# ivanalberico/End-To-End-Self-Supervised-SLAM

Hardware: AMD Instinct MI355X
Metric: online refinement steps/sec @640x480, seq_len=60 (higher is better)
Workload: dtype f32

## Files before the change

end-to-end-self-supervised-slam_amd/csrc/conv.hip:

```cpp
#include <cassert>
#include <type_traits>

#include "e2e_common.h"

typedef float f4v __attribute__((ext_vector_type(4)));
typedef float f16v __attribute__((ext_vector_type(16)));

#define CBK 16

enum { ACT_NONE = 0, ACT_RELU = 1, ACT_ELU = 2, ACT_DISP = 3 };

struct ConvArgs {
    const float* src0;
    const float* src1;
    const float* w;
    const float* scale;
    const float* shift;
    const float* res;
    float* out;
    int B, Hs, Ws;
    int Cin, C1, up;
    int Hd, Wd;
    int Ncols, ldw;
    int KH, KW, stride, pad, pad_mode;
    int off;
    int act;
    float in_sub, in_mul;
    int ksplit, cps;
    float* slab;
    int cls;
    const float* xin;
    int dact;
    const float* pre;
    int64_t cls_rows;
    int64_t bytes0, bytes1, bytesw;
};

__device__ __forceinline__ float apply_act(float v, int act) {
    if (act == ACT_RELU) return fmaxf(v, 0.f);
    if (act == ACT_ELU) return v > 0.f ? v : expm1f(v);
    if (act == ACT_DISP) return 10.f / (1.f + expf(-v)) + 0.01f;
    return v;
}

__device__ __forceinline__ float act_deriv(float y, int act) {
    if (act == ACT_RELU) return y > 0.f ? 1.f : 0.f;
    if (act == ACT_ELU) return y > 0.f ? 1.f : y + 1.f;
    return 1.f;
}

template <bool TRANSPOSED>
__device__ __forceinline__ bool tap_coord(const ConvArgs& a, int yd, int xd, int kh, int kw, int& ys, int& xs) {
    if (!TRANSPOSED) {
        ys = yd * a.stride + kh - a.pad;
        xs = xd * a.stride + kw - a.pad;
        if (a.pad_mode == 1) {
            ys = reflect1(ys, a.Hs);
            xs = reflect1(xs, a.Ws);
// ... 821 lines not shown
    float wreg[9][KQ];
#pragma unroll
    for (int t = 0; t < 9; ++t)
#pragma unroll
        for (int j = 0; j < KQ; ++j) wreg[t][j] = a.w[(int64_t)((a.flip ? 8 - t : t) * CIN + 4 * j + kq) * a.ldw + l16];
    const float* sb = a.src + (int64_t)b * a.Hsrc * a.Wsrc * CIN;
    for (int idx = tid; idx < PH * PW * KQ; idx += 256) {
        const int q = (UP == 2) ? idx / (PH * PW) : idx % KQ, pix = (UP == 2) ? idx % (PH * PW) : idx / KQ;
        const int py = pix / PW, px = pix - py * PW;
        int Y = y0 - a.org + py, X = x0 - a.org + px;
        bool ok = true;
        if (REFLECT) {
            Y = min(max(reflect1(Y, HD), 0), HD - 1);
            X = min(max(reflect1(X, WD), 0), WD - 1);
        } else {
            ok = Y >= 0 && Y < HD && X >= 0 && X < WD;
        }
        f4v v = {0.f, 0.f, 0.f, 0.f};
        if (ok) v = *(const f4v*)(sb + ((int64_t)(Y / UP) * a.Wsrc + (X / UP)) * CIN + q * 4);
#pragma unroll
        for (int e = 0; e < 4; ++e) patch[(q * 4 + e) * PLANE + py * PWS + px] = v[e];
    }
    __syncthreads();
    const float bv = a.bias ? a.bias[l16] : 0.f;
    float* ob = a.out + (int64_t)b * a.Hd * a.Wd * 16;
#pragma unroll 1
    for (int g2 = 0; g2 < TH; g2 += 2) {
        const int g0 = wave * TH + g2, g1 = g0 + 1;
        const int r0 = g0 >> 2, c0 = (g0 & 3) * 16, r1 = g1 >> 2, c1 = (g1 & 3) * 16;
        f4v acc0 = {0.f, 0.f, 0.f, 0.f}, acc1 = {0.f, 0.f, 0.f, 0.f};
        const float* p0 = patch + kq * PLANE + r0 * PWS + c0 + l16;
        const float* p1 = patch + kq * PLANE + r1 * PWS + c1 + l16;
#pragma unroll
        for (int t = 0; t < 9; ++t) {
            const int off = (t / 3) * PWS + (t % 3);
#pragma unroll
            for (int j = 0; j < KQ; ++j) {
                acc0 = __builtin_amdgcn_mfma_f32_16x16x4f32(p0[4 * j * PLANE + off], wreg[t][j], acc0, 0, 0, 0);
                acc1 = __builtin_amdgcn_mfma_f32_16x16x4f32(p1[4 * j * PLANE + off], wreg[t][j], acc1, 0, 0, 0);
            }
        }
#pragma unroll
        for (int h = 0; h < 2; ++h) {
            const f4v acc = h ? acc1 : acc0;
            const int y = y0 + (h ? r1 : r0), xb = x0 + (h ? c1 : c0) + 4 * kq;
            if (y >= a.Hd) continue;
#pragma unroll
            for (int i = 0; i < 4; ++i)
                if (xb + i < a.Wd) ob[((int64_t)y * a.Wd + xb + i) * 16 + l16] = apply_act(acc[i] + bv, a.act);
        }
    }
}

struct StemArgs {
    const float* src;
    const float* w;
    const float* scale;
    const float* shift;
    float* out;
    int B, Hs, Ws, Hd, Wd, ldw, act;
    float in_sub, in_mul;
};

__global__ __launch_bounds__(256) void k_conv7x7_stem(StemArgs a) {
    constexpr int TH = 4, TW = 32, PH = 2 * TH + 6, PW = 2 * TW + 5, ROW = 208, NJ = 37;
    __shared__ float patch[PH * ROW];
    const int tid = threadIdx.x, lane = tid & 63, wave = tid >> 6, l16 = lane & 15, kq = lane >> 4;
    const int x0 = blockIdx.x * TW, y0 = blockIdx.y * TH, b = blockIdx.z;
    const int co = 16 * wave + l16;
    float wreg[NJ];
    int offk[NJ];
#pragma unroll
    for (int j = 0; j < NJ; ++j) {
        const int k = 4 * j + kq;
        wreg[j] = k < 147 ? a.w[(int64_t)k * a.ldw + co] : 0.f;
        offk[j] = k + (k / 21) * (ROW - 21);
    }
    const float* sb = a.src + (int64_t)b * a.Hs * a.Ws * 3;
    for (int idx = tid; idx < PH * ROW; idx += 256) {
        const int py = idx / ROW, e = idx - py * ROW;
        const int Y = 2 * y0 - 3 + py, X = 2 * x0 - 3 + e / 3;
        const bool ok = e < 3 * PW && Y >= 0 && Y < a.Hs && X >= 0 && X < a.Ws;
        patch[idx] = ok ? (sb[((int64_t)Y * a.Ws + X) * 3 + (e - (e / 3) * 3)] - a.in_sub) * a.in_mul : 0.f;
    }
    __syncthreads();
    const float sc = a.scale ? a.scale[co] : 1.f, sh = a.shift ? a.shift[co] : 0.f;
    float* ob = a.out + (int64_t)b * a.Hd * a.Wd * 64;
#pragma unroll 1
    for (int g = 0; g < 2 * TH; g += 2) {
        const int r = g >> 1;
        const float* p0 = patch + 2 * r * ROW + 6 * l16;
        const float* p1 = p0 + 6 * 16;
        f4v acc0 = {0.f, 0.f, 0.f, 0.f}, acc1 = {0.f, 0.f, 0.f, 0.f};
#pragma unroll
        for (int j = 0; j < NJ; ++j) {
            acc0 = __builtin_amdgcn_mfma_f32_16x16x4f32(p0[offk[j]], wreg[j], acc0, 0, 0, 0);
            acc1 = __builtin_amdgcn_mfma_f32_16x16x4f32(p1[offk[j]], wreg[j], acc1, 0, 0, 0);
        }
        const int y = y0 + r;
        if (y >= a.Hd) continue;
#pragma unroll
        for (int h = 0; h < 2; ++h) {
            const f4v acc = h ? acc1 : acc0;
            const int xb = x0 + 16 * h + 4 * kq;
#pragma unroll
            for (int i = 0; i < 4; ++i)
// ... 1850 lines not shown
}

int64_t e2e_conv_tuned_workspace_floats(int64_t rows, int cols) {
    int64_t n = (int64_t)16 * rows * cols;
    if (n < (int64_t)SK_MAX_G * 64 * 64) n = (int64_t)SK_MAX_G * 64 * 64;
    return n + SK_FLAG_FLOATS;
}
int e2e_conv_workspace_flag_floats(void) { return SK_FLAG_FLOATS; }
int e2e_conv_streamk_error_index(void) { return SK_ERR_INDEX; }

int e2e_conv_gemm_choice(int64_t rows, int cols, int K, int chunk_depth, int allow_split, int* out3) {
    E2E_REQUIRE(out3 && rows > 0 && cols > 0 && K > 0 && (chunk_depth == 16 || chunk_depth == 32), E2E_ERR_ARG, "e2e_conv_gemm_choice: bad argument");
    const GemmCfg c = choose_cfg(rows, cols, K, chunk_depth, allow_split != 0);
    out3[0] = c.bm; out3[1] = c.bn; out3[2] = c.S;
    return E2E_OK;
}

struct ConvGeom { int B, Hs, Ws, Cin, Cout, Ho, Wo, KH, KW, stride, pad, pad_mode, C1, up; float in_sub, in_mul; };
#define GEOM_LAYER(g) ConvGeom g{}; g.B = B; g.Hs = Hs; g.Ws = Ws; g.Cin = Cin; g.Cout = Cout; g.KH = KH; g.KW = KW; g.stride = stride; g.pad = pad; g.pad_mode = pad_mode
#define GEOM_SOURCES(g) g.C1 = C1; g.up = up; g.in_sub = in_sub; g.in_mul = in_mul
#define GEOM_OUTPUT(g) g.Ho = Ho; g.Wo = Wo
#define GEOM_BWD_DATA(g) GEOM_LAYER(g); GEOM_OUTPUT(g)
#define GEOM_BWD_WEIGHT(g) GEOM_LAYER(g); GEOM_OUTPUT(g); GEOM_SOURCES(g)
#define GEOM_WGRAD_QUERY(g) ConvGeom g{}; g.B = B; g.Ho = Ho; g.Wo = Wo; g.Cin = Cin; g.Cout = Cout; g.KH = KH; g.KW = KW
struct FwdOps { const float *src0, *src1, *w_fwd; int ld_fwd; const float *scale, *shift, *residual; float* out; int act; };
struct BwdDataOps { const float* dz; const float* w_bwd; int ld_bwd; float* dxp; int accumulate; const float* x_in; int in_act; const float* pre_add; };
struct WgradIn { const float *dz, *src0, *src1; float* workspace; };

static int fwd_setup(const FwdOps& f, const ConvGeom& g, ConvArgs& a_out, int& vec_out, const char* who) {
    const int B = g.B, Hs = g.Hs, Ws = g.Ws, Cin = g.Cin, Cout = g.Cout, KH = g.KH, KW = g.KW, stride = g.stride, pad = g.pad, pad_mode = g.pad_mode;
    const int C1 = g.C1, up = g.up, ld_fwd = f.ld_fwd;
    E2E_REQUIRE(f.src0 && f.w_fwd && f.out && B > 0 && Hs > 0 && Ws > 0 && Cin > 0 && Cout > 0 && KH > 0 && KW > 0, E2E_ERR_ARG, "%s: bad argument", who);
    E2E_REQUIRE(up == 1 || up == 2, E2E_ERR_ARG, "%s: upsample factor must be 1 or 2", who);
    E2E_REQUIRE(C1 > 0 && C1 <= Cin && (C1 == Cin || f.src1), E2E_ERR_ARG, "%s: bad channel split", who);
    E2E_REQUIRE(pad_mode == 0 || (pad_mode == 1 && pad == 1 && Hs >= 2 && Ws >= 2), E2E_ERR_ARG, "%s: reflection padding needs pad == 1", who);
    E2E_REQUIRE(stride == 1 || stride == 2, E2E_ERR_ARG, "%s: stride must be 1 or 2", who);
    E2E_REQUIRE(Hs % up == 0 && Ws % up == 0 && ld_fwd % 4 == 0 && ld_fwd >= Cout, E2E_ERR_ARG, "%s: bad sizes", who);
    E2E_REQUIRE(pad >= 0 && Hs + 2 * pad >= KH && Ws + 2 * pad >= KW, E2E_ERR_ARG, "%s: the kernel must fit the padded input (pad >= 0)", who);
    const int vec = (Cin % 16 == 0 && (C1 == Cin || C1 % 16 == 0)) ? 4 : 1;
    E2E_REQUIRE(vec == 4 || (C1 == Cin && up == 1), E2E_ERR_ARG, "%s: the scalar path (Cin %% 16 != 0) takes a single full-resolution source", who);
    E2E_REQUIRE((int64_t)B * Hs * Ws * Cin * 4 < (1ll << 30) && (int64_t)KH * KW * Cin * ld_fwd * 4 < (1ll << 31), E2E_ERR_ARG,
                "%s: activations must stay below 1 GB, weights below 2 GB (32-bit buffer offsets with out-of-range markers)", who);
    E2E_REQUIRE(vec != 4 || (KH <= 3 && KW <= 3), E2E_ERR_ARG, "%s: the channel-quad loader takes kernels up to 3 x 3", who);
    ConvArgs a{};
    a.src0 = f.src0; a.src1 = f.src1; a.w = f.w_fwd; a.scale = f.scale; a.shift = f.shift; a.res = f.residual; a.out = f.out;
    a.B = B; a.Hs = Hs; a.Ws = Ws; a.Cin = Cin; a.C1 = C1; a.up = up;
    a.Hd = (Hs + 2 * pad - KH) / stride + 1; a.Wd = (Ws + 2 * pad - KW) / stride + 1;
    a.Ncols = Cout; a.ldw = ld_fwd; a.KH = KH; a.KW = KW; a.stride = stride; a.pad = pad; a.pad_mode = pad_mode; a.off = 0; a.act = f.act;
    a.in_sub = g.in_sub; a.in_mul = g.in_mul;
    a_out = a; vec_out = vec;
    return E2E_OK;
}

static int conv_fwd_impl(const FwdOps& f, const ConvGeom& g, float* workspace, GemmCfg force, void* stream) {
    const int B = g.B, Hs = g.Hs, Ws = g.Ws, Cin = g.Cin, Cout = g.Cout, KH = g.KH, KW = g.KW, stride = g.stride, pad = g.pad, pad_mode = g.pad_mode;
    const int C1 = g.C1, up = g.up, ld_fwd = f.ld_fwd;
    ConvArgs a;
    int vec;
    const int rc = fwd_setup(f, g, a, vec, "e2e_conv2d_fwd");
    if (rc != E2E_OK) return rc;
    if (!force.bm && KH == 7 && KW == 7 && stride == 2 && pad == 3 && pad_mode == 0 && Cin == 3 && Cout == 64 && C1 == Cin && up == 1 && !f.residual && ld_fwd >= 64) {
        StemArgs t{f.src0, f.w_fwd, f.scale, f.shift, f.out, B, Hs, Ws, a.Hd, a.Wd, ld_fwd, f.act, g.in_sub, g.in_mul};
        hipLaunchKernelGGL(k_conv7x7_stem, dim3((a.Wd + 31) / 32, (a.Hd + 3) / 4, B), dim3(256), 0, (hipStream_t)stream, t);
    }
    else if (!force.bm && KH == 3 && KW == 3 && stride == 1 && pad == 1 && pad_mode == 1 && Cout == 16 && C1 == Cin && !f.scale && !f.residual && ld_fwd >= 16 &&
        ((Cin == 16 && up == 2) || (Cin == 32 && up == 1))) {
        ThinArgs t{f.src0, f.w_fwd, f.shift, f.out, B, Hs / up, Ws / up, Hs, Ws, ld_fwd, f.act, 1, 0};
        if (Cin == 16) hipLaunchKernelGGL((k_conv3x3_thin<16, 2, true, 8>), dim3((Ws + 63) / 64, (Hs + 7) / 8, B), dim3(256), 0, (hipStream_t)stream, t);
        else hipLaunchKernelGGL((k_conv3x3_thin<32, 1, true, 4>), dim3((Ws + 63) / 64, (Hs + 3) / 4, B), dim3(256), 0, (hipStream_t)stream, t);
    } else
        launch_gemm<false>(a, vec, workspace, force, (hipStream_t)stream);
    E2E_LAUNCH_CHECK("e2e_conv2d_fwd");
    return E2E_OK;
}

int e2e_conv2d_fwd(const float* src0, const float* src1, int C1, int up, const float* w_fwd, int ld_fwd, const float* scale,
                   const float* shift, const float* residual, float* out, int B, int Hs, int Ws, int Cin, int Cout, int KH,
                   int KW, int stride, int pad, int pad_mode, int act, float in_sub, float in_mul, float* workspace, void* stream) {
    GEOM_LAYER(g); GEOM_SOURCES(g);
    return conv_fwd_impl(FwdOps{src0, src1, w_fwd, ld_fwd, scale, shift, residual, out, act}, g, workspace, GemmCfg{0, 0, 0}, stream);
}

static bool tuning_ok(int tile_m, int tile_n, int ksplit) {
    if (tile_m == 0) return true;
    if (ksplit < 0) return tile_m == 64 && tile_n == 64 && -ksplit <= SK_MAX_G;
    return tile_max_cb(tile_m, tile_n) != 0 && ksplit >= 1 && ksplit <= 16;
}

int e2e_conv2d_fwd_tuned(const float* src0, const float* src1, int C1, int up, const float* w_fwd, int ld_fwd, const float* scale,
                         const float* shift, const float* residual, float* out, int B, int Hs, int Ws, int Cin, int Cout, int KH,
                         int KW, int stride, int pad, int pad_mode, int act, float in_sub, float in_mul, float* workspace, int tile_m, int tile_n,
                         int ksplit, void* stream) {
    E2E_REQUIRE(tuning_ok(tile_m, tile_n, ksplit), E2E_ERR_ARG, "e2e_conv2d_fwd_tuned: unsupported decomposition %d x %d / %d", tile_m, tile_n, ksplit);
    GEOM_LAYER(g); GEOM_SOURCES(g);
    return conv_fwd_impl(FwdOps{src0, src1, w_fwd, ld_fwd, scale, shift, residual, out, act}, g, workspace, GemmCfg{tile_m, tile_n, ksplit}, stream);
}

struct EntryOps {
    const float* x;
    const float *w1_fwd; int ld1; const float *scale1, *shift1; float* out1; int act1; float* workspace1;
    const float* wd_fwd; int ldd; const float *gamma, *beta, *mean, *var; float eps; float *bn_scale, *bn_shift, *bn_rstd, *z, *y;
};
struct EntryPlan { ConvArgs a1, ad; int vec1, vecd; GemmLaunch p1, pd; ConvGeom g1, gd; bool paired; };

static int fwd_entry_plan(const EntryOps& q, const ConvGeom& g, EntryPlan& P, const char* who) {
    E2E_REQUIRE(q.gamma && q.beta && q.mean && q.var && q.bn_scale && q.bn_shift && q.bn_rstd && q.z && q.y, E2E_ERR_ARG, "%s: bad argument", who);
    E2E_REQUIRE(g.pad_mode == 0 && g.C1 == g.Cin && g.up == 1, E2E_ERR_ARG, "%s: a stage entry reads one zero-padded full-resolution source", who);
    P.g1 = g;
    P.gd = g; P.gd.KH = P.gd.KW = 1; P.gd.pad = 0;
    int rc = fwd_setup(FwdOps{q.x, nullptr, q.w1_fwd, q.ld1, q.scale1, q.shift1, nullptr, q.out1, q.act1}, P.g1, P.a1, P.vec1, who);
    if (rc != E2E_OK) return rc;
    rc = fwd_setup(FwdOps{q.x, nullptr, q.wd_fwd, q.ldd, nullptr, nullptr, nullptr, q.z, ACT_NONE}, P.gd, P.ad, P.vecd, who);
    if (rc != E2E_OK) return rc;
    E2E_REQUIRE(P.a1.Hd == P.ad.Hd && P.a1.Wd == P.ad.Wd, E2E_ERR_ARG, "%s: the two branches must produce the same output grid", who);
    P.paired = false;
    if (P.vec1 != 4 || P.vecd != 4 || g.Cout < 128) return E2E_OK;
    P.p1 = plan_gemm<false>(P.a1, 4, q.workspace1, GemmCfg{0, 0, 0});
    P.pd = plan_gemm<false>(P.ad, 4, nullptr, GemmCfg{0, 0, 0});
    auto t14 = [](const GemmLaunch& p) { return p.kind == GK_TILE && p.cb == 32 && p.c.bm == 32 && p.c.bn == 128; };
    P.paired = t14(P.p1) && t14(P.pd) && P.pd.tail == GT_NONE && P.ad.ksplit == 1 && P.pd.g.z == 1;
    return E2E_OK;
// ... 90 lines not shown
    return bwd_data_impl(BwdDataOps{dz, w_bwd, ld_bwd, dxp, 0, nullptr, 0, nullptr}, g, workspace, stream);
}

int e2e_conv2d_bwd_data_acc(const float* dz, const float* w_bwd, int ld_bwd, float* dxp, int B, int Hs, int Ws, int Cin, int Cout,
                            int Ho, int Wo, int KH, int KW, int stride, int pad, int pad_mode, int accumulate, float* workspace,
                            void* stream) {
    GEOM_BWD_DATA(g);
    return bwd_data_impl(BwdDataOps{dz, w_bwd, ld_bwd, dxp, accumulate, nullptr, 0, nullptr}, g, workspace, stream);
}

int e2e_conv2d_bwd_data_fused(const float* da, const float* w_bwd, int ld_bwd, float* dxp, int B, int Hs, int Ws, int Cin, int Cout,
                              int Ho, int Wo, int KH, int KW, int stride, int pad, int pad_mode, int accumulate, const float* x_in,
                              int in_act, const float* pre_add, float* workspace, void* stream) {
    GEOM_BWD_DATA(g);
    return bwd_data_impl(BwdDataOps{da, w_bwd, ld_bwd, dxp, accumulate, x_in, in_act, pre_add}, g, workspace, stream);
}

int e2e_conv2d_bwd_data_fused_tuned(const float* da, const float* w_bwd, int ld_bwd, float* dxp, int B, int Hs, int Ws, int Cin, int Cout,
                                    int Ho, int Wo, int KH, int KW, int stride, int pad, int pad_mode, int accumulate, const float* x_in,
                                    int in_act, const float* pre_add, float* workspace, int tile_m, int tile_n, int ksplit, void* stream) {
    E2E_REQUIRE(tuning_ok(tile_m, tile_n, ksplit), E2E_ERR_ARG, "e2e_conv2d_bwd_data_fused_tuned: unsupported decomposition %d x %d / %d", tile_m, tile_n, ksplit);
    GEOM_BWD_DATA(g);
    return bwd_data_impl(BwdDataOps{da, w_bwd, ld_bwd, dxp, accumulate, x_in, in_act, pre_add}, g, workspace, stream, GemmCfg{tile_m, tile_n, ksplit});
}

struct GatherAdjoint { const float* dxp; int B, Hs, Ws, Cin, C1, up, padded; float *d0, *d1; int acc0, acc1; const float* x0; int act0; const float* x1; int act1; };
static void launch_gather_adjoint(const GatherAdjoint& q, hipStream_t st) {
    const int64_t n = (int64_t)q.B * (q.Hs / q.up) * (q.Ws / q.up) * q.C1 + (int64_t)q.B * q.Hs * q.Ws * (q.Cin - q.C1);
    if (q.Cin % 4 == 0 && q.C1 % 4 == 0 && n < (1ll << 31))
        hipLaunchKernelGGL(k_gather_adjoint4, dim3(egrid(n / 4)), dim3(256), 0, st, q.dxp, q.B, q.Hs, q.Ws, q.Cin, q.C1, q.up, q.padded ? 1 : 0, q.d0, q.d1, q.acc0, q.acc1,
                           q.x0, q.act0, q.x1, q.act1);
    else
        hipLaunchKernelGGL(k_gather_adjoint, dim3(egrid(n)), dim3(256), 0, st, q.dxp, q.B, q.Hs, q.Ws, q.Cin, q.C1, q.up, q.padded ? 1 : 0, q.d0, q.d1, q.acc0, q.acc1,
                           q.x0, q.act0, q.x1, q.act1);
}

int e2e_conv2d_gather_adjoint(const float* dxp, int B, int Hs, int Ws, int Cin, int C1, int up, int padded, float* d_src0,
                              float* d_src1, int accumulate0, int accumulate1, void* stream) {
    E2E_REQUIRE(dxp && d_src0 && B > 0 && Cin > 0 && C1 > 0 && C1 <= Cin && (C1 == Cin || d_src1) && (up == 1 || up == 2), E2E_ERR_ARG,
                "e2e_conv2d_gather_adjoint: bad argument");
    launch_gather_adjoint(GatherAdjoint{dxp, B, Hs, Ws, Cin, C1, up, padded, d_src0, d_src1, accumulate0, accumulate1, nullptr, 0, nullptr, 0}, (hipStream_t)stream);
    E2E_LAUNCH_CHECK("e2e_conv2d_gather_adjoint");
    return E2E_OK;
}

int e2e_conv2d_gather_adjoint_act(const float* dxp, int B, int Hs, int Ws, int Cin, int C1, int up, int padded, float* d_src0, float* d_src1,
                                  int accumulate0, int accumulate1, const float* src0, int act0, const float* src1, int act1, void* stream) {
    E2E_REQUIRE(dxp && d_src0 && B > 0 && Cin > 0 && C1 > 0 && C1 <= Cin && (C1 == Cin || d_src1) && (up == 1 || up == 2), E2E_ERR_ARG,
                "e2e_conv2d_gather_adjoint_act: bad argument");
    E2E_REQUIRE((act0 == 0 || src0) && (act1 == 0 || src1) && act0 >= 0 && act0 <= 2 && act1 >= 0 && act1 <= 2, E2E_ERR_ARG,
                "e2e_conv2d_gather_adjoint_act: an activation derivative needs the activation's output");
    launch_gather_adjoint(GatherAdjoint{dxp, B, Hs, Ws, Cin, C1, up, padded, d_src0, d_src1, accumulate0, accumulate1, src0, act0, src1, act1}, (hipStream_t)stream);
    E2E_LAUNCH_CHECK("e2e_conv2d_gather_adjoint_act");
    return E2E_OK;
}

int e2e_conv2d_act_bwd(const float* dy, const float* y, const float* scale, float* dz, int64_t n, int C, int act, void* stream) {
    E2E_REQUIRE(dy && y && dz && n > 0 && C > 0 && act >= 0 && act <= 3, E2E_ERR_ARG, "e2e_conv2d_act_bwd: bad argument");
    hipLaunchKernelGGL(k_act_bwd, dim3(egrid(n)), dim3(256), 0, (hipStream_t)stream, dy, y, scale, dz, n, C, act, 0);
    E2E_LAUNCH_CHECK("e2e_conv2d_act_bwd");
    return E2E_OK;
}

int e2e_conv2d_act_bwd_acc(const float* dy, const float* y, const float* scale, float* dz, int64_t n, int C, int act, int accumulate,
                           void* stream) {
    E2E_REQUIRE(dy && y && dz && n > 0 && C > 0 && act >= 0 && act <= 3, E2E_ERR_ARG, "e2e_conv2d_act_bwd_acc: bad argument");
    hipLaunchKernelGGL(k_act_bwd, dim3(egrid(n)), dim3(256), 0, (hipStream_t)stream, dy, y, scale, dz, n, C, act, accumulate);
    E2E_LAUNCH_CHECK("e2e_conv2d_act_bwd_acc");
    return E2E_OK;
}

#define HEAD_PARTS 2048
int e2e_head_fwd(const float* x, const float* w, const float* bias, float* y, int B, int H, int W, int Cin, int act, void* stream) {
    E2E_REQUIRE(x && w && y && B > 0 && H >= 2 && W >= 2 && Cin == HC, E2E_ERR_ARG, "e2e_head_fwd: bad argument (the head takes %d channels)", HC);
    hipLaunchKernelGGL(k_head_fwd, dim3(egrid((int64_t)B * H * W * 4)), dim3(256), 0, (hipStream_t)stream, x, w, bias, y, B, H, W, act);
    E2E_LAUNCH_CHECK("e2e_head_fwd");
    return E2E_OK;
}
int64_t e2e_head_workspace_floats(void) { return (int64_t)HEAD_PARTS * (9 * HC + 1); }
int e2e_head_bwd_act(const float* dz, const float* x, const float* w, float* dx, float* dw, float* dbias, float* workspace, int B, int H,
                     int W, int Cin, int in_act, void* stream) {
    E2E_REQUIRE(dz && x && w && workspace && B > 0 && H >= 2 && W >= 2 && Cin == HC && in_act >= 0 && in_act <= 2, E2E_ERR_ARG, "e2e_head_bwd: bad argument");
    E2E_REQUIRE((int64_t)B * H * W * HC < (1ll << 31), E2E_ERR_ARG, "e2e_head_bwd: activation too large for 32-bit element offsets");
    hipStream_t st = (hipStream_t)stream;
    const char* ev = getenv("E2E_HEAD_BWD_FUSED");
    if (dx && dw && !(ev && ev[0] == '0')) {
        hipLaunchKernelGGL(k_head_bwd_fused, dim3(HEAD_PARTS), dim3(256), 0, st, dz, x, w, dx, workspace, B, H, W, in_act);
        hipLaunchKernelGGL(k_head_wreduce, dim3(9 * HC + 1), dim3(256), 0, st, workspace, HEAD_PARTS, dw, dbias);
        E2E_LAUNCH_CHECK("e2e_head_bwd");
        return E2E_OK;
    }
    if (dx) hipLaunchKernelGGL(k_head_bwd_data, dim3(egrid((int64_t)B * H * W * 4)), dim3(256), 0, st, dz, w, dx, B, H, W, x, in_act);
    if (dw) {
        hipLaunchKernelGGL(k_head_bwd_weight, dim3(HEAD_PARTS), dim3(256), 0, st, dz, x, workspace, B, H, W);
        hipLaunchKernelGGL(k_head_wreduce, dim3(9 * HC + 1), dim3(256), 0, st, workspace, HEAD_PARTS, dw, dbias);
    }
    E2E_LAUNCH_CHECK("e2e_head_bwd");
    return E2E_OK;
}

int e2e_head_bwd(const float* dz, const float* x, const float* w, float* dx, float* dw, float* dbias, float* workspace, int B, int H,
                 int W, int Cin, void* stream) {
    return e2e_head_bwd_act(dz, x, w, dx, dw, dbias, workspace, B, H, W, Cin, 0, stream);
}

enum WgradPath { WP_STEM, WP_THIN, WP_TAPS, WP_GEMM16, WP_GEMM_LEAN, WP_GEMM, WP_COUNT };
// ... 355 lines not shown
```

end-to-end-self-supervised-slam_amd/e2ehip/netplan.py:

```python
import ctypes
import os

import torch

from . import _lib as L
from .conv import ACT, _ld, epoch_sum

_f32 = torch.float32
PAIR_WGRAD_FIRST = 0
PAIR_CARRY_PLACE = 0


class Buf:
    __slots__ = ("t", "g", "written", "B", "h", "w", "C", "act")

    def __init__(self, B, h, w, C, dev, need_grad=True, act=0):
        self.B, self.h, self.w, self.C = B, h, w, C
        self.act = act
        self.t = torch.empty(B, h, w, C, device=dev, dtype=_f32)
        self.g = torch.empty(B, h, w, C, device=dev, dtype=_f32) if need_grad else None
        self.written = False

    def nchw(self):
        return self.t.permute(0, 3, 1, 2)


def _at(t, slot):
    return L.ptr(t if slot is None else t[slot])


def _sink_of(p):
    s = getattr(p, "_e2e_grad_sink", None)
    if s is None:
        if p.grad is None:
            p.grad = torch.zeros_like(p)
        s = p.grad
    return s


class _Conv:
    def __init__(self, plan, src0, src1, weight, bias, bn, residual, act, stride, pad, pad_mode, up, in_norm):
        dev = plan.dev
        self.src0, self.src1, self.res = src0, src1, residual
        self.weight, self.bias = weight, bias
        self.Cout, self.Cin, self.KH, self.KW = weight.shape
        self.C1 = src0.C
        if self.C1 + (src1.C if src1 is not None else 0) != self.Cin:
            raise ValueError("channel mismatch in the launch plan")
        self.up, self.stride, self.pad, self.pm, self.act = up, stride, pad, 1 if pad_mode == "reflect" else 0, ACT[act]
        self.isub, self.imul = in_norm if in_norm is not None else (0.0, 1.0)
        B = src0.B
        self.Hs, self.Ws = src0.h * up, src0.w * up
        self.Ho, self.Wo = (self.Hs + 2 * pad - self.KH) // stride + 1, (self.Ws + 2 * pad - self.KW) // stride + 1
        if self.act not in (0, ACT["relu"], ACT["elu"]):
            raise NotImplementedError("launch plan: convolution epilogues are none / ReLU / ELU (the sigmoid head has its own op)")
        self.out = Buf(B, self.Ho, self.Wo, self.Cout, dev, act=self.act)
        self.ldf, self.ldb = _ld(self.Cout), _ld(self.Cin)
        self.wf = torch.zeros(self.KH * self.KW * self.Cin, self.ldf, device=dev, dtype=_f32)
        self.need_dx = src0.g is not None
        self.wb = torch.zeros(self.KH * self.KW * self.Cout, self.ldb, device=dev, dtype=_f32) if self.need_dx else None
        self.scale = self.shift = None
        if bn is not None:
            w, b, rm, rv, eps = bn
            with torch.no_grad():
                self.scale = (w / torch.sqrt(rv + eps)).contiguous()
                self.shift = (b - rm * self.scale).contiguous()
        self.geom = dict(B=B, Hs=self.Hs, Ws=self.Ws, Cin=self.Cin, Cout=self.Cout, Ho=self.Ho, Wo=self.Wo, KH=self.KH, KW=self.KW, stride=stride,
                         pad=pad, pad_mode=self.pm, C1=self.C1, up=up, in_sub=float(self.isub), in_mul=float(self.imul))
        n = max(L.query("e2e_conv2d_splitk_workspace_floats", b * self.Ho * self.Wo, self.Cout, self.KH * self.KW * self.Cin) for b in {B, 1})
        self.ws_f = torch.zeros(n, device=dev, dtype=_f32) if n else None
        self.pp = pad if self.pm == 1 else 0
        self.direct = self.pp == 0 and up == 1 and src1 is None
        if self.need_dx:
            n = L.query("e2e_conv2d_bwd_data_workspace_floats", geom=self.geom, Hd=self.Hs + 2 * self.pp, Wd=self.Ws + 2 * self.pp, cols=self.Cin,
                        K=self.KH * self.KW * self.Cout)
            self.ws_b = torch.zeros(n, device=dev, dtype=_f32) if n else None
            self.dxp = None if self.direct else torch.empty(B, self.Hs + 2 * self.pp, self.Ws + 2 * self.pp, self.Cin, device=dev, dtype=_f32)
        self.ws_w = torch.empty(L.query("e2e_conv2d_wgrad_workspace_floats", geom=self.geom, has_bias=1 if bias is not None else 0), device=dev, dtype=_f32)
        self.res_via, self.res_aliased, self.pre_from = None, False, None
        self.entry, self.fwd_in = None, None
        self.reduce_desc = L.WgradReduceDesc()

    def layout_row(self):
        return [self.weight.data_ptr(), self.wf.data_ptr(), self.wb.data_ptr() if self.wb is not None else 0, self.Cout, self.Cin, self.KH, self.KW,
                self.ldf, self.ldb, self.scale.data_ptr() if (self.scale is not None and self.wb is not None) else 0]

    def fwd(self, plan, st, slot=None):
        s = self
        if s.fwd_in is not None:
            return
        if s.entry is not None:
            ds, bn = s.entry
            b = bn.bn
            L.call("e2e_conv2d_fwd_entry_pair", geom=s.geom, B=s.src0.B if slot is None else 1, x=_at(s.src0.t, slot), w1_fwd=L.ptr(s.wf), ld1=s.ldf,
                   scale1=L.ptr(s.scale), shift1=L.ptr(s.shift), out1=_at(s.out.t, slot), act1=s.act, workspace1=L.ptr(s.ws_f), wd_fwd=L.ptr(ds.wf),
                   ldd=ds.ldf, gamma=L.ptr(b.weight), beta=L.ptr(b.bias), running_mean=L.ptr(b.running_mean), running_var=L.ptr(b.running_var),
                   eps=float(b.eps), bn_scale=L.ptr(bn.scale), bn_shift=L.ptr(bn.shift), bn_rstd=L.ptr(bn.rstd), z=_at(ds.out.t, slot),
                   y=_at(bn.out.t, slot), stream=st)
            return
        L.call("e2e_conv2d_fwd", geom=s.geom, B=s.src0.B if slot is None else 1, src0=_at(s.src0.t, slot),
               src1=_at(s.src1.t, slot) if s.src1 is not None else None, w_fwd=L.ptr(s.wf), ld_fwd=s.ldf, scale=L.ptr(s.scale),
               shift=L.ptr(s.shift if s.bias is None else s.bias), residual=_at(s.res.t, slot) if s.res is not None else None,
               out=_at(s.out.t, slot), act=s.act, workspace=L.ptr(s.ws_f), stream=st)

    def bwd(self, plan, st):
        s = self
        n = s.out.t.numel()
        g = s.out.g
        if s.res is not None and s.res_via is None and not s.res_aliased:
            L.call("e2e_conv2d_act_bwd_acc", L.ptr(g), L.ptr(s.res.t), None, L.ptr(s.res.g), n, s.Cout, s.res.act, 1 if s.res.written else 0, st)
            s.res.written = True
        if s.need_dx and plan.paired and not plan.overlap:
            pre = s.pre_from.out.g if (s.direct and s.pre_from is not None) else None
            acc, in_act = (1 if s.src0.written else 0) if s.direct else 0, s.src0.act if s.direct else 0
            carry = plan.carry_for(s, lambda: L.query("e2e_conv2d_bwd_pair_is_one_launch", geom=s.geom, ld_bwd=s.ldb, accumulate=acc, in_act=in_act,
                                                      has_pre_add=1 if pre is not None else 0, has_workspace=1 if s.ws_b is not None else 0,
                                                      has_src1=1 if s.src1 is not None else 0, has_bias=1 if s.bias is not None else 0))
            L.call("e2e_conv2d_bwd_pair_carry" if carry else "e2e_conv2d_bwd_pair_deferred", geom=s.geom, da=L.ptr(g), w_bwd=L.ptr(s.wb), ld_bwd=s.ldb,
                   dxp=L.ptr(s.src0.g if s.direct else s.dxp), accumulate=acc, x_in=L.ptr(s.src0.t) if s.direct else None, in_act=in_act, pre_add=L.ptr(pre),
                   workspace=L.ptr(s.ws_b), workspace_w=L.ptr(s.ws_w), accumulate_w=0, wgrad_first=PAIR_WGRAD_FIRST, stream=st, **s._wgrad_operands(plan),
                   **(carry or {}))
            if s.direct:
                s.src0.written = True
            else:
                self._gather_adjoint(st)
            return
        if s.need_dx:
            if s.direct:
                pre = s.pre_from.out.g if s.pre_from is not None else None
                L.call("e2e_conv2d_bwd_data_fused", geom=s.geom, da=L.ptr(g), w_bwd=L.ptr(s.wb), ld_bwd=s.ldb, dxp=L.ptr(s.src0.g),
                       accumulate=1 if s.src0.written else 0, x_in=L.ptr(s.src0.t), in_act=s.src0.act, pre_add=L.ptr(pre), workspace=L.ptr(s.ws_b), stream=st)
                s.src0.written = True
            else:
                L.call("e2e_conv2d_bwd_data", geom=s.geom, dz=L.ptr(g), w_bwd=L.ptr(s.wb), ld_bwd=s.ldb, dxp=L.ptr(s.dxp), workspace=L.ptr(s.ws_b), stream=st)
                self._gather_adjoint(st)
        plan.carry_for(s, None)
        st_w = plan.fork(st)
        L.call("e2e_conv2d_bwd_weight_scaled_deferred", geom=s.geom, da=L.ptr(g), workspace=L.ptr(s.ws_w), accumulate=0, stream=st_w, **s._wgrad_operands(plan))

    def _wgrad_operands(self, plan):
        s = self
        return dict(out_scale=L.ptr(s.scale), src0=L.ptr(s.src0.t), src1=L.ptr(s.src1.t) if s.src1 is not None else None, dw=L.ptr(plan.sink(s.weight)),
                    dbias=L.ptr(plan.sink(s.bias)) if s.bias is not None else None, desc_out_host=ctypes.byref(s.reduce_desc))

    def _gather_adjoint(self, st):
        s, s1 = self, self.src1
        L.call("e2e_conv2d_gather_adjoint_act", geom=s.geom, dxp=L.ptr(s.dxp), padded=1 if s.pp else 0, d_src0=L.ptr(s.src0.g),
               d_src1=L.ptr(s1.g) if s1 is not None else None, accumulate0=1 if s.src0.written else 0,
               accumulate1=1 if (s1 is not None and s1.written) else 0, src0=L.ptr(s.src0.t), act0=s.src0.act,
               src1=L.ptr(s1.t) if s1 is not None else None, act1=s1.act if s1 is not None else 0, stream=st)
        s.src0.written = True
        if s1 is not None:
            s1.written = True


class _Head:

    def __init__(self, plan, src, weight, bias, act):
        self.src, self.weight, self.bias, self.act = src, weight, bias, ACT[act]
        self.out = Buf(src.B, src.h, src.w, 1, plan.dev)
        self.dz = torch.empty_like(self.out.t)
        self.ws = torch.empty(L.load().e2e_head_workspace_floats(), device=plan.dev, dtype=_f32)

    def fwd(self, plan, st, slot=None):
        s = self.src
        L.call("e2e_head_fwd", _at(s.t, slot), L.ptr(self.weight), L.ptr(self.bias), _at(self.out.t, slot), s.B if slot is None else 1, s.h, s.w, s.C, self.act, st)

    def bwd(self, plan, st):
        s, n = self.src, self.out.t.numel()
        L.call("e2e_conv2d_act_bwd", L.ptr(self.out.g), L.ptr(self.out.t), None, L.ptr(self.dz), n, 1, self.act, st)
        if s.written:
            raise RuntimeError("the disparity head's input has a single consumer")
        L.call("e2e_head_bwd_act", dz=L.ptr(self.dz), x=L.ptr(s.t), w=L.ptr(self.weight), dx=L.ptr(s.g), dw=L.ptr(plan.sink(self.weight)),
               dbias=L.ptr(plan.sink(self.bias)) if self.bias is not None else None, workspace=L.ptr(self.ws), B=s.B, H=s.h, W=s.w, Cin=s.C,
               in_act=s.act, stream=st)
        s.written = True


class _MaxPool:
    def __init__(self, plan, src):
# ... 343 lines not shown
```

include/e2eslam.h:

```cpp
#ifndef E2ESLAM_H
#define E2ESLAM_H

#include <stdint.h>

#ifdef __cplusplus
extern "C" {
#endif

#define E2E_OK 0
#define E2E_ERR_ARG (-1)
#define E2E_ERR_LAUNCH (-2)
#define E2E_ERR_WORKSPACE (-3)

#define E2E_PADDING_ZEROS 0
#define E2E_PADDING_BORDER 1

typedef struct e2e_strides {
    int64_t sb, sc, sh, sw;
} e2e_strides;

int e2e_version(void);
const char* e2e_last_error(void);


// ... 228 lines not shown

int e2e_conv_weight_layouts(const float* w, int Cout, int Cin, int KH, int KW, float* w_fwd,
                            int ld_fwd, float* w_bwd, int ld_bwd, void* stream);

int e2e_conv_weight_layouts_batched(const long long* desc, int nlayers, void* stream);

int e2e_conv2d_fwd(const float* src0, const float* src1, int C1, int up, const float* w_fwd,
                   int ld_fwd, const float* scale, const float* shift, const float* residual,
                   float* out, int B, int Hs, int Ws, int Cin, int Cout, int KH, int KW, int stride,
                   int pad, int pad_mode, int act, float in_sub, float in_mul, float* workspace,
                   void* stream);
int64_t e2e_conv2d_splitk_workspace_floats(int64_t rows, int cols, int K);
int64_t e2e_conv2d_bwd_data_workspace_floats(int B, int Hd, int Wd, int cols, int K, int stride);
int e2e_conv_workspace_flag_floats(void);
int e2e_conv_streamk_error_index(void);
int64_t e2e_conv_tuned_workspace_floats(int64_t rows, int cols);
int e2e_conv2d_fwd_tuned(const float* src0, const float* src1, int C1, int up, const float* w_fwd, int ld_fwd, const float* scale,
                         const float* shift, const float* residual, float* out, int B, int Hs, int Ws, int Cin, int Cout, int KH,
                         int KW, int stride, int pad, int pad_mode, int act, float in_sub, float in_mul, float* workspace, int tile_m,
                         int tile_n, int ksplit, void* stream);
int e2e_conv2d_bwd_data_fused_tuned(const float* da, const float* w_bwd, int ld_bwd, float* dxp, int B, int Hs, int Ws, int Cin, int Cout,
                                    int Ho, int Wo, int KH, int KW, int stride, int pad, int pad_mode, int accumulate, const float* x_in,
                                    int in_act, const float* pre_add, float* workspace, int tile_m, int tile_n, int ksplit, void* stream);
int64_t e2e_conv2d_wgrad_tuned_workspace_floats(int B, int Ho, int Wo, int Cin, int Cout, int KH, int KW, int has_bias, int target_workgroups);
int e2e_conv2d_bwd_weight_scaled_tuned(const float* da, const float* out_scale, const float* src0, const float* src1, int C1, int up,
                                       float* dw, float* dbias, float* workspace, int B, int Hs, int Ws, int Cin, int Cout, int Ho, int Wo,
                                       int KH, int KW, int stride, int pad, int pad_mode, int accumulate, float in_sub, float in_mul,
                                       int target_workgroups, void* stream);
int e2e_conv_gemm_choice(int64_t rows, int cols, int K, int chunk_depth, int allow_split, int* out3_host);

int e2e_conv2d_act_bwd(const float* dy, const float* y, const float* scale, float* dz, int64_t n,
                       int C, int act, void* stream);
int e2e_conv2d_act_bwd_acc(const float* dy, const float* y, const float* scale, float* dz, int64_t n,
                           int C, int act, int accumulate, void* stream);

int e2e_conv2d_bwd_data(const float* dz, const float* w_bwd, int ld_bwd, float* dxp, int B, int Hs,
                        int Ws, int Cin, int Cout, int Ho, int Wo, int KH, int KW, int stride,
                        int pad, int pad_mode, float* workspace, void* stream);
int e2e_conv2d_bwd_data_acc(const float* dz, const float* w_bwd, int ld_bwd, float* dxp, int B, int Hs,
                            int Ws, int Cin, int Cout, int Ho, int Wo, int KH, int KW, int stride,
                            int pad, int pad_mode, int accumulate, float* workspace, void* stream);
int e2e_conv2d_bwd_data_fused(const float* da, const float* w_bwd, int ld_bwd, float* dxp, int B, int Hs,
                              int Ws, int Cin, int Cout, int Ho, int Wo, int KH, int KW, int stride,
                              int pad, int pad_mode, int accumulate, const float* x_in, int in_act,
                              const float* pre_add, float* workspace, void* stream);
int e2e_conv2d_gather_adjoint(const float* dxp, int B, int Hs, int Ws, int Cin, int C1, int up,
                              int padded, float* d_src0, float* d_src1, int accumulate0,
                              int accumulate1, void* stream);

int e2e_conv2d_gather_adjoint_act(const float* dxp, int B, int Hs, int Ws, int Cin, int C1, int up,
                                  int padded, float* d_src0, float* d_src1, int accumulate0,
                                  int accumulate1, const float* src0, int act0, const float* src1,
                                  int act1, void* stream);

int64_t e2e_conv2d_wgrad_workspace_floats(int B, int Ho, int Wo, int Cin, int Cout, int KH, int KW,
                                          int has_bias);
int e2e_conv2d_bwd_weight(const float* dz, const float* src0, const float* src1, int C1, int up,
                          float* dw, float* dbias, float* workspace, int B, int Hs, int Ws, int Cin,
                          int Cout, int Ho, int Wo, int KH, int KW, int stride, int pad,
                          int pad_mode, int accumulate, float in_sub, float in_mul, void* stream);

int e2e_conv2d_bwd_weight_scaled(const float* da, const float* out_scale, const float* src0,
                                 const float* src1, int C1, int up, float* dw, float* dbias,
                                 float* workspace, int B, int Hs, int Ws, int Cin, int Cout, int Ho,
                                 int Wo, int KH, int KW, int stride, int pad, int pad_mode,
                                 int accumulate, float in_sub, float in_mul, void* stream);

typedef struct e2e_wgrad_reduce_desc {
    const float* slabs;
    float* dw;
    float* dbias;
    const float* scale;
    int S, Mpad, Npad, Cout, Cin, KH, KW, has_bias, accumulate;
    int zl;
    long long first_item;
} e2e_wgrad_reduce_desc;
int e2e_conv2d_bwd_weight_scaled_deferred(const float* da, const float* out_scale, const float* src0,
                                          const float* src1, int C1, int up, float* dw, float* dbias,
                                          float* workspace, int B, int Hs, int Ws, int Cin, int Cout, int Ho,
                                          int Wo, int KH, int KW, int stride, int pad, int pad_mode,
                                          int accumulate, float in_sub, float in_mul,
                                          e2e_wgrad_reduce_desc* desc_out_host, void* stream);
int e2e_conv2d_bwd_pair_deferred(const float* da, const float* w_bwd, int ld_bwd, float* dxp, int B, int Hs,
                                 int Ws, int Cin, int Cout, int Ho, int Wo, int KH, int KW, int stride,
                                 int pad, int pad_mode, int accumulate, const float* x_in, int in_act,
                                 const float* pre_add, float* workspace, const float* out_scale,
                                 const float* src0, const float* src1, int C1, int up, float* dw,
                                 float* dbias, float* workspace_w, int accumulate_w, float in_sub,
                                 float in_mul, e2e_wgrad_reduce_desc* desc_out_host, int wgrad_first,
                                 void* stream);
int e2e_conv2d_bwd_pair_carry(const float* da, const float* w_bwd, int ld_bwd, float* dxp, int B, int Hs,
                              int Ws, int Cin, int Cout, int Ho, int Wo, int KH, int KW, int stride,
                              int pad, int pad_mode, int accumulate, const float* x_in, int in_act,
                              const float* pre_add, float* workspace, const float* out_scale,
                              const float* src0, const float* src1, int C1, int up, float* dw,
                              float* dbias, float* workspace_w, int accumulate_w, float in_sub,
                              float in_mul, e2e_wgrad_reduce_desc* desc_out_host, int wgrad_first,
                              const e2e_wgrad_reduce_desc* carry_descs_dev, int carry_n,
                              long long carry_first_item, long long carry_items, int carry_place,
                              void* stream);
int e2e_conv2d_bwd_pair_is_one_launch(int ld_bwd, int B, int Hs, int Ws, int Cin, int Cout, int Ho, int Wo,
                                      int KH, int KW, int stride, int pad, int pad_mode, int accumulate,
                                      int in_act, int has_pre_add, int has_workspace, int has_src1, int C1,
                                      int up, int has_bias);
int e2e_conv2d_fwd_entry_pair(const float* x, const float* w1_fwd, int ld1, const float* scale1, const float* shift1,
                              float* out1, int act1, float* workspace1, const float* wd_fwd, int ldd,
// ... 132 lines not shown
```

Before: 225.2.

## Add polyphase 3x3 conv kernels for x2-upsampled 16-channel layers

Adds phase-decomposed kernels for a 3x3 reflection-padded conv that follows a nearest x2 upsample with 16 channels. The forward kernel folds the weights per output phase into 2x2 taps on the low-resolution input, and the backward-data kernel writes the low-resolution input gradient directly, applying the activation derivative and handling reflection-border corrections. This removes the padded full-resolution dx buffer and the separate gather-adjoint launch. The forward path is opt-in through an environment variable, while the backward path is on by default, which adds border-correction complexity.

```diff
diff --git a/end-to-end-self-supervised-slam_amd/csrc/conv.hip b/end-to-end-self-supervised-slam_amd/csrc/conv.hip
--- a/end-to-end-self-supervised-slam_amd/csrc/conv.hip
+++ b/end-to-end-self-supervised-slam_amd/csrc/conv.hip
@@ -4,6 +4,7 @@
 #include "e2e_common.h"
 
 typedef float f4v __attribute__((ext_vector_type(4)));
+typedef float f2v __attribute__((ext_vector_type(2)));
 typedef float f16v __attribute__((ext_vector_type(16)));
 
 #define CBK 16
@@ -931,6 +932,178 @@
     }
 }
 
+struct Up2Args {
+    const float* src;
+    const float* w;
+    const float* bias;
+    float* out;
+    int B, Hl, Wl, ldw, act;
+};
+
+__global__ __launch_bounds__(256) void k_conv3x3_up2_phase(Up2Args a) {
+    constexpr int C = 16, TH = 8, TW = 64, PH = TH / 2 + 2, PW = TW / 2 + 2, PWS = 40, PLANE = PH * PWS, KQ = C / 4;
+    static_assert(PLANE % 32 == 16 && PWS >= PW, "the two channel planes a half-wave reads must sit 16 banks apart");
+    __shared__ float patch[C * PLANE];
+    const int tid = threadIdx.x, lane = tid & 63, wave = tid >> 6, l16 = lane & 15, kq = lane >> 4;
+    const int x0 = blockIdx.x * TW, y0 = blockIdx.y * TH, b = blockIdx.z;
+    const int Hd = 2 * a.Hl, Wd = 2 * a.Wl;
+    const int py = wave & 1, half = wave >> 1;
+    float wreg[2][2][2][KQ];
+#pragma unroll
+    for (int j = 0; j < KQ; ++j) {
+        float w9[9];
+#pragma unroll
+        for (int t = 0; t < 9; ++t) w9[t] = a.w[(int64_t)(t * C + 4 * j + kq) * a.ldw + l16];
+#pragma unroll
+        for (int ta = 0; ta < 2; ++ta) {
+            float r[3];
+#pragma unroll
+            for (int kw = 0; kw < 3; ++kw)
+                r[kw] = ta == 0 ? (py ? w9[kw] + w9[3 + kw] : w9[kw]) : (py ? w9[6 + kw] : w9[3 + kw] + w9[6 + kw]);
+            wreg[0][ta][0][j] = r[0];
+            wreg[0][ta][1][j] = r[1] + r[2];
+            wreg[1][ta][0][j] = r[0] + r[1];
+            wreg[1][ta][1][j] = r[2];
+        }
+    }
+    const float* sb = a.src + (int64_t)b * a.Hl * a.Wl * C;
+    const int m0 = y0 / 2 - 1, n0 = x0 / 2 - 1;
+    for (int idx = tid; idx < PH * PW * KQ; idx += 256) {
+        const int q = idx % KQ, pix = idx / KQ;
+        const int pr = pix / PW, pc = pix - pr * PW;
+        const int R = min(max(m0 + pr, 0), a.Hl - 1), Cc = min(max(n0 + pc, 0), a.Wl - 1);
+        const f4v v = *(const f4v*)(sb + ((int64_t)R * a.Wl + Cc) * C + q * 4);
+#pragma unroll
+        for (int e = 0; e < 4; ++e) patch[(q * 4 + e) * PLANE + pr * PWS + pc] = v[e];
+    }
+    __syncthreads();
+    const float bv = a.bias ? a.bias[l16] : 0.f;
+    float* ob = a.out + (int64_t)b * Hd * Wd * 16;
+#pragma unroll 1
+    for (int k = 0; k < TH / 2; ++k) {
+        const int y = y0 + 2 * k + py;
+        const float* p = patch + kq * PLANE + (k + py) * PWS + half * 16 + l16;
+        f4v acc0 = {0.f, 0.f, 0.f, 0.f}, acc1 = {0.f, 0.f, 0.f, 0.f};
+#pragma unroll
+        for (int ta = 0; ta < 2; ++ta)
+#pragma unroll
+            for (int j = 0; j < KQ; ++j) {
+                const float* pj = p + 4 * j * PLANE + ta * PWS;
+                const float v0 = pj[0], v1 = pj[1], v2 = pj[2];
+                acc0 = __builtin_amdgcn_mfma_f32_16x16x4f32(v0, wreg[0][ta][0][j], acc0, 0, 0, 0);
+                acc1 = __builtin_amdgcn_mfma_f32_16x16x4f32(v1, wreg[1][ta][0][j], acc1, 0, 0, 0);
+                acc0 = __builtin_amdgcn_mfma_f32_16x16x4f32(v1, wreg[0][ta][1][j], acc0, 0, 0, 0);
+                acc1 = __builtin_amdgcn_mfma_f32_16x16x4f32(v2, wreg[1][ta][1][j], acc1, 0, 0, 0);
+            }
+        if (y >= Hd) continue;
+        const int xb = x0 + 2 * (half * 16 + 4 * kq);
+#pragma unroll
+        for (int i = 0; i < 4; ++i) {
+            const int x = xb + 2 * i;
+            if (x < Wd) {
+                float* o = ob + ((int64_t)y * Wd + x) * 16 + l16;
+                o[0] = apply_act(acc0[i] + bv, a.act);
+                o[16] = apply_act(acc1[i] + bv, a.act);
+            }
+        }
+    }
+}
+
+struct Up2BwdArgs {
+    const float* dz;
+    const float* w;
+    const float* src;
+    float* dsrc;
+    int B, Hl, Wl, ldw, act, accumulate;
+};
+
+__global__ __launch_bounds__(256) void k_conv3x3_up2_phase_bwd(Up2BwdArgs a) {
+    constexpr int C = 16, BH = 4, BW = 32, PH = 2 * BH + 2, PW = 2 * BW + 2, PWS = PW, PLANE = 672, KQ = C / 4;
+    static_assert(PLANE % 64 == 32 && PLANE >= PH * PWS && PWS % 2 == 0, "8-byte reads: the two channel planes a half-wave reads must sit 32 banks apart");
+    __shared__ __attribute__((aligned(16))) float patch[C * PLANE];
+    const int tid = threadIdx.x, lane = tid & 63, wave = tid >> 6, l16 = lane & 15, kq = lane >> 4;
+    const int n0 = blockIdx.x * BW, m0 = blockIdx.y * BH, b = blockIdx.z;
+    const int Hd = 2 * a.Hl, Wd = 2 * a.Wl;
+    float wb[4][4][KQ];
+#pragma unroll
+    for (int j = 0; j < KQ; ++j) {
+        float w9[9];
+#pragma unroll
+        for (int t = 0; t < 9; ++t) w9[t] = a.w[(int64_t)(t * C + 4 * j + kq) * a.ldw + l16];
+#pragma unroll
+        for (int u = 0; u < 4; ++u) {
+            float r[3];
+#pragma unroll
+            for (int kw = 0; kw < 3; ++kw) r[kw] = u == 0 ? w9[6 + kw] : u == 1 ? w9[3 + kw] + w9[6 + kw] : u == 2 ? w9[kw] + w9[3 + kw] : w9[kw];
+            wb[u][0][j] = r[2];
+            wb[u][1][j] = r[1] + r[2];
+            wb[u][2][j] = r[0] + r[1];
+            wb[u][3][j] = r[0];
+        }
+    }
+    const float* zb = a.dz + (int64_t)b * Hd * Wd * C;
+#pragma unroll 2
+    for (int idx = tid; idx < PH * PW * KQ; idx += 256) {
+        const int q = idx % KQ, pix = idx / KQ;
+        const int pr = pix / PW, pc = pix - pr * PW;
+        const int Y = 2 * m0 - 1 + pr, X = 2 * n0 - 1 + pc;
+        f4v v = {0.f, 0.f, 0.f, 0.f};
+        if (Y >= 0 && Y < Hd && X >= 0 && X < Wd) v = *(const f4v*)(zb + ((int64_t)Y * Wd + X) * C + q * 4);
+#pragma unroll
+        for (int e = 0; e < 4; ++e) patch[(q * 4 + e) * PLANE + pr * PWS + pc] = v[e];
+    }
+    __syncthreads();
+    const int m = m0 + wave;
+    if (m >= a.Hl) return;
+    const bool top = m == 0, bottom = m == a.Hl - 1;
+    const bool left = n0 == 0;
+    const int er = a.Wl - 1 - n0;
+    const bool right0 = er >= 0 && er < 16, right1 = er >= 16 && er < 32;
+    const bool lane_l = l16 == 0, lane_r = l16 == (er & 15);
+    f4v acc0 = {0.f, 0.f, 0.f, 0.f}, acc1 = {0.f, 0.f, 0.f, 0.f};
+    const float* p = patch + kq * PLANE + 2 * wave * PWS + 2 * l16;
+    auto row_tap = [&](auto ua_c, auto uw_c) {
+        constexpr int ua = decltype(ua_c)::value, uw = decltype(uw_c)::value;
+#pragma unroll
+        for (int j = 0; j < KQ; ++j) {
+            const float* pj = p + 4 * j * PLANE + ua * PWS;
+            const f2v a01 = *(const f2v*)pj, a23 = *(const f2v*)(pj + 2), b01 = *(const f2v*)(pj + 32), b23 = *(const f2v*)(pj + 34);
+            acc0 = __builtin_amdgcn_mfma_f32_16x16x4f32(a01[0], wb[uw][0][j], acc0, 0, 0, 0);
+            acc1 = __builtin_amdgcn_mfma_f32_16x16x4f32(b01[0], wb[uw][0][j], acc1, 0, 0, 0);
+            acc0 = __builtin_amdgcn_mfma_f32_16x16x4f32(a01[1], wb[uw][1][j], acc0, 0, 0, 0);
+            acc1 = __builtin_amdgcn_mfma_f32_16x16x4f32(b01[1], wb[uw][1][j], acc1, 0, 0, 0);
+            acc0 = __builtin_amdgcn_mfma_f32_16x16x4f32(a23[0], wb[uw][2][j], acc0, 0, 0, 0);
+            acc1 = __builtin_amdgcn_mfma_f32_16x16x4f32(b23[0], wb[uw][2][j], acc1, 0, 0, 0);
+            acc0 = __builtin_amdgcn_mfma_f32_16x16x4f32(a23[1], wb[uw][3][j], acc0, 0, 0, 0);
+            acc1 = __builtin_amdgcn_mfma_f32_16x16x4f32(b23[1], wb[uw][3][j], acc1, 0, 0, 0);
+            if (left) acc0 = __builtin_amdgcn_mfma_f32_16x16x4f32(lane_l ? a01[1] : 0.f, wb[uw][3][j], acc0, 0, 0, 0);
+            if (right0) acc0 = __builtin_amdgcn_mfma_f32_16x16x4f32(lane_r ? a23[0] : 0.f, wb[uw][0][j], acc0, 0, 0, 0);
+            if (right1) acc1 = __builtin_amdgcn_mfma_f32_16x16x4f32(lane_r ? b23[0] : 0.f, wb[uw][0][j], acc1, 0, 0, 0);
+        }
+    };
+    using std::integral_constant;
+    row_tap(integral_constant<int, 0>{}, integral_constant<int, 0>{});
+    row_tap(integral_constant<int, 1>{}, integral_constant<int, 1>{});
+    row_tap(integral_constant<int, 2>{}, integral_constant<int, 2>{});
+    row_tap(integral_constant<int, 3>{}, integral_constant<int, 3>{});
+    if (top) row_tap(integral_constant<int, 1>{}, integral_constant<int, 3>{});
+    if (bottom) row_tap(integral_constant<int, 2>{}, integral_constant<int, 0>{});
+    const int64_t rowb = ((int64_t)b * a.Hl + m) * a.Wl;
+#pragma unroll
+    for (int h = 0; h < 2; ++h) {
+        const f4v acc = h ? acc1 : acc0;
+#pragma unroll
+        for (int i = 0; i < 4; ++i) {
+            const int n = n0 + 16 * h + 4 * kq + i;
+            if (n >= a.Wl) continue;
+            const int64_t e = (rowb + n) * C + l16;
+            float s = acc[i];
+            if (a.act) s *= act_deriv(a.src[e], a.act);
+            a.dsrc[e] = a.accumulate ? a.dsrc[e] + s : s;
+        }
+    }
+}
+
 struct StemArgs {
     const float* src;
     const float* w;
@@ -2887,6 +3060,11 @@
     return E2E_OK;
 }
 
+static bool up2_phase_forward() {
+    const char* ev = getenv("E2E_UP2_PHASE");
+    return ev && (ev[0] == '1' || ev[0] == 'f');
+}
+
 static int conv_fwd_impl(const FwdOps& f, const ConvGeom& g, float* workspace, GemmCfg force, void* stream) {
     const int B = g.B, Hs = g.Hs, Ws = g.Ws, Cin = g.Cin, Cout = g.Cout, KH = g.KH, KW = g.KW, stride = g.stride, pad = g.pad, pad_mode = g.pad_mode;
     const int C1 = g.C1, up = g.up, ld_fwd = f.ld_fwd;
@@ -2901,7 +3079,10 @@
     else if (!force.bm && KH == 3 && KW == 3 && stride == 1 && pad == 1 && pad_mode == 1 && Cout == 16 && C1 == Cin && !f.scale && !f.residual && ld_fwd >= 16 &&
         ((Cin == 16 && up == 2) || (Cin == 32 && up == 1))) {
         ThinArgs t{f.src0, f.w_fwd, f.shift, f.out, B, Hs / up, Ws / up, Hs, Ws, ld_fwd, f.act, 1, 0};
-        if (Cin == 16) hipLaunchKernelGGL((k_conv3x3_thin<16, 2, true, 8>), dim3((Ws + 63) / 64, (Hs + 7) / 8, B), dim3(256), 0, (hipStream_t)stream, t);
+        if (Cin == 16 && up2_phase_forward()) {
+            Up2Args u{f.src0, f.w_fwd, f.shift, f.out, B, Hs / 2, Ws / 2, ld_fwd, f.act};
+            hipLaunchKernelGGL(k_conv3x3_up2_phase, dim3((Ws + 63) / 64, (Hs + 7) / 8, B), dim3(256), 0, (hipStream_t)stream, u);
+        } else if (Cin == 16) hipLaunchKernelGGL((k_conv3x3_thin<16, 2, true, 8>), dim3((Ws + 63) / 64, (Hs + 7) / 8, B), dim3(256), 0, (hipStream_t)stream, t);
         else hipLaunchKernelGGL((k_conv3x3_thin<32, 1, true, 4>), dim3((Ws + 63) / 64, (Hs + 3) / 4, B), dim3(256), 0, (hipStream_t)stream, t);
     } else
         launch_gemm<false>(a, vec, workspace, force, (hipStream_t)stream);
@@ -3098,6 +3279,31 @@
                 "e2e_conv2d_gather_adjoint_act: an activation derivative needs the activation's output");
     launch_gather_adjoint(GatherAdjoint{dxp, B, Hs, Ws, Cin, C1, up, padded, d_src0, d_src1, accumulate0, accumulate1, src0, act0, src1, act1}, (hipStream_t)stream);
     E2E_LAUNCH_CHECK("e2e_conv2d_gather_adjoint_act");
+    return E2E_OK;
+}
+
+static bool up2_phase_geometry(const ConvGeom& g) {
+    return g.KH == 3 && g.KW == 3 && g.stride == 1 && g.pad == 1 && g.pad_mode == 1 && g.up == 2 && g.C1 == 16 && g.Cin == 16 && g.Cout == 16 && g.B > 0 &&
+           g.Hs >= 2 && g.Ws >= 2 && g.Hs % 2 == 0 && g.Ws % 2 == 0 && g.Ho == g.Hs && g.Wo == g.Ws && (int64_t)g.B * g.Hs * g.Ws * 16 * 4 < (1ll << 30);
+}
+
+int e2e_conv2d_bwd_data_up2_is_direct(int ld_bwd, int B, int Hs, int Ws, int Cin, int Cout, int Ho, int Wo, int KH, int KW, int stride, int pad,
+                                      int pad_mode, int C1, int up) {
+    GEOM_BWD_DATA(g); g.C1 = C1; g.up = up;
+    return up2_phase_geometry(g) && ld_bwd >= 16 && ld_bwd % 4 == 0 ? 1 : 0;
+}
+
+int e2e_conv2d_bwd_data_up2_act(const float* dz, const float* w_bwd, int ld_bwd, float* d_src0, int B, int Hs, int Ws, int Cin, int Cout, int Ho,
+                                int Wo, int KH, int KW, int stride, int pad, int pad_mode, int C1, int up, int accumulate0, const float* src0,
+                                int act0, void* stream) {
+    E2E_REQUIRE(dz && w_bwd && d_src0 && (act0 == 0 || src0) && act0 >= 0 && act0 <= 2, E2E_ERR_ARG,
+                "e2e_conv2d_bwd_data_up2_act: bad argument (an activation derivative needs the activation's output)");
+    E2E_REQUIRE(e2e_conv2d_bwd_data_up2_is_direct(ld_bwd, B, Hs, Ws, Cin, Cout, Ho, Wo, KH, KW, stride, pad, pad_mode, C1, up), E2E_ERR_ARG,
+                "e2e_conv2d_bwd_data_up2_act: serves 3x3 / stride 1 / reflection pad 1 behind a x2 upsample, 16 -> 16 channels (e2e_conv2d_bwd_data_up2_is_direct)");
+    const int Hl = Hs / 2, Wl = Ws / 2;
+    Up2BwdArgs t{dz, w_bwd, src0, d_src0, B, Hl, Wl, ld_bwd, act0, accumulate0 ? 1 : 0};
+    hipLaunchKernelGGL(k_conv3x3_up2_phase_bwd, dim3((Wl + 31) / 32, (Hl + 3) / 4, B), dim3(256), 0, (hipStream_t)stream, t);
+    E2E_LAUNCH_CHECK("e2e_conv2d_bwd_data_up2_act");
     return E2E_OK;
 }
 
diff --git a/end-to-end-self-supervised-slam_amd/e2ehip/netplan.py b/end-to-end-self-supervised-slam_amd/e2ehip/netplan.py
--- a/end-to-end-self-supervised-slam_amd/e2ehip/netplan.py
+++ b/end-to-end-self-supervised-slam_amd/e2ehip/netplan.py
@@ -71,11 +71,13 @@
         self.ws_f = torch.zeros(n, device=dev, dtype=_f32) if n else None
         self.pp = pad if self.pm == 1 else 0
         self.direct = self.pp == 0 and up == 1 and src1 is None
+        self.up2 = False
         if self.need_dx:
             n = L.query("e2e_conv2d_bwd_data_workspace_floats", geom=self.geom, Hd=self.Hs + 2 * self.pp, Wd=self.Ws + 2 * self.pp, cols=self.Cin,
                         K=self.KH * self.KW * self.Cout)
             self.ws_b = torch.zeros(n, device=dev, dtype=_f32) if n else None
-            self.dxp = None if self.direct else torch.empty(B, self.Hs + 2 * self.pp, self.Ws + 2 * self.pp, self.Cin, device=dev, dtype=_f32)
+            self.up2 = src1 is None and bool(L.query("e2e_conv2d_bwd_data_up2_is_direct", geom=self.geom, ld_bwd=self.ldb))
+            self.dxp = None if (self.direct or self._up2_now()) else self._dxp_buffer()
         self.ws_w = torch.empty(L.query("e2e_conv2d_wgrad_workspace_floats", geom=self.geom, has_bias=1 if bias is not None else 0), device=dev, dtype=_f32)
         self.res_via, self.res_aliased, self.pre_from = None, False, None
         self.entry, self.fwd_in = None, None
@@ -84,6 +86,12 @@
     def layout_row(self):
         return [self.weight.data_ptr(), self.wf.data_ptr(), self.wb.data_ptr() if self.wb is not None else 0, self.Cout, self.Cin, self.KH, self.KW,
                 self.ldf, self.ldb, self.scale.data_ptr() if (self.scale is not None and self.wb is not None) else 0]
+
+    def _up2_now(self):
+        return self.up2 and os.environ.get("E2E_UP2_PHASE", "b")[:1] in ("", "1", "b")
+
+    def _dxp_buffer(self):
+        return torch.empty(self.src0.B, self.Hs + 2 * self.pp, self.Ws + 2 * self.pp, self.Cin, device=self.src0.t.device, dtype=_f32)
 
     def fwd(self, plan, st, slot=None):
         s = self
@@ -110,7 +118,13 @@
         if s.res is not None and s.res_via is None and not s.res_aliased:
             L.call("e2e_conv2d_act_bwd_acc", L.ptr(g), L.ptr(s.res.t), None, L.ptr(s.res.g), n, s.Cout, s.res.act, 1 if s.res.written else 0, st)
             s.res.written = True
-        if s.need_dx and plan.paired and not plan.overlap:
+        if s.need_dx and s._up2_now():
+            L.call("e2e_conv2d_bwd_data_up2_act", geom=s.geom, dz=L.ptr(g), w_bwd=L.ptr(s.wb), ld_bwd=s.ldb, d_src0=L.ptr(s.src0.g),
+                   accumulate0=1 if s.src0.written else 0, src0=L.ptr(s.src0.t), act0=s.src0.act, stream=st)
+            s.src0.written = True
+        elif s.need_dx and plan.paired and not plan.overlap:
+            if s.dxp is None and not s.direct:
+                s.dxp = s._dxp_buffer()
             pre = s.pre_from.out.g if (s.direct and s.pre_from is not None) else None
             acc, in_act = (1 if s.src0.written else 0) if s.direct else 0, s.src0.act if s.direct else 0
             carry = plan.carry_for(s, lambda: L.query("e2e_conv2d_bwd_pair_is_one_launch", geom=s.geom, ld_bwd=s.ldb, accumulate=acc, in_act=in_act,
@@ -125,7 +139,9 @@
             else:
                 self._gather_adjoint(st)
             return
-        if s.need_dx:
+        elif s.need_dx:
+            if s.dxp is None and not s.direct:
+                s.dxp = s._dxp_buffer()
             if s.direct:
                 pre = s.pre_from.out.g if s.pre_from is not None else None
                 L.call("e2e_conv2d_bwd_data_fused", geom=s.geom, da=L.ptr(g), w_bwd=L.ptr(s.wb), ld_bwd=s.ldb, dxp=L.ptr(s.src0.g),
diff --git a/include/e2eslam.h b/include/e2eslam.h
--- a/include/e2eslam.h
+++ b/include/e2eslam.h
@@ -304,6 +304,13 @@
                                   int padded, float* d_src0, float* d_src1, int accumulate0,
                                   int accumulate1, const float* src0, int act0, const float* src1,
                                   int act1, void* stream);
+
+int e2e_conv2d_bwd_data_up2_is_direct(int ld_bwd, int B, int Hs, int Ws, int Cin, int Cout, int Ho, int Wo,
+                                      int KH, int KW, int stride, int pad, int pad_mode, int C1, int up);
+int e2e_conv2d_bwd_data_up2_act(const float* dz, const float* w_bwd, int ld_bwd, float* d_src0, int B, int Hs,
+                                int Ws, int Cin, int Cout, int Ho, int Wo, int KH, int KW, int stride,
+                                int pad, int pad_mode, int C1, int up, int accumulate0, const float* src0,
+                                int act0, void* stream);
 
 int64_t e2e_conv2d_wgrad_workspace_floats(int B, int Ho, int Wo, int Cin, int Cout, int KH, int KW,
                                           int has_bias);
```

Result: no change. 226.2 (median of 6 runs) (+0.4%).
